# Plachtaa/VALL-E-X

Hardware: AMD Instinct MI355X
Metric: audio-seconds/sec (AR+NAR+Vocos end to end; AR codec-tokens/sec in ar_tokens_per_s), batch32 8s utt (higher is better)
Workload: dtype f32 (cached AR decode step) + f16x2 (operands split into fp16 head + tail = 22 significant bits, tail x tail dropped, fp32 accumulate) for the prefill / NAR projections and full-sequence attention

## Files before the change

### vall-e-x_amd/csrc/engine.hip

```cpp
#include "engine_ctx.h"

#include <deque>
#include <memory>

namespace {
thread_local std::string g_create_err;
}

namespace vxe {

const float* W(vx_ctx* c, const std::string& name) {
  auto it = c->w.find(name);
  return it == c->w.end() ? nullptr : it->second.d;
}

static int ring_slot(vx_ctx* c, size_t n, char** slot) {
  PinRing& r = c->ring;
  if (!r.base) FAIL(VX_ESTATE, "the context has no pinned transfer ring");
  const size_t a = (n + 255) & ~(size_t)255;
  if (r.head + a > r.cap) if (int e = xfer_sync(c)) return e;
  *slot = r.base + r.head;
  r.head += a;
  return VX_OK;
}

int xfer_h2d(vx_ctx* c, void* dst_dev, const void* src_host, size_t bytes) {
  const char* s = static_cast<const char*>(src_host);
  char* d = static_cast<char*>(dst_dev);
  while (bytes) {
    const size_t n = std::min(bytes, XFER_CHUNK);
    char* slot = nullptr;
    if (int e = ring_slot(c, n, &slot)) return e;
    memcpy(slot, s, n);
    HIPCHK(hipMemcpyAsync(d, slot, n, hipMemcpyHostToDevice, c->stream));
    s += n; d += n; bytes -= n;
  }
  return VX_OK;
}

int xfer_d2h(vx_ctx* c, void* dst_host, const void* src_dev, size_t bytes) {
  char* d = static_cast<char*>(dst_host);
  const char* s = static_cast<const char*>(src_dev);
  while (bytes) {
    const size_t n = std::min(bytes, XFER_CHUNK);
    char* slot = nullptr;
    if (int e = ring_slot(c, n, &slot)) return e;
    HIPCHK(hipMemcpyAsync(slot, s, n, hipMemcpyDeviceToHost, c->stream));
    c->ring.pend.push_back({d, slot, n});
    s += n; d += n; bytes -= n;
  }
  return VX_OK;
}

int xfer_sync(vx_ctx* c) {
  const hipError_t e = hipStreamSynchronize(c->stream);
  PinRing& r = c->ring;
  if (e == hipSuccess) {
    size_t total = 0;
    for (const PinRing::Pend& p : r.pend) total += p.n;
    if (total < ((size_t)4 << 20)) {
      for (const PinRing::Pend& p : r.pend) memcpy(p.dst, p.src, p.n);
    } else {
      struct Piece { char* dst; const char* src; size_t n; };
      std::vector<Piece> pieces;
      for (const PinRing::Pend& p : r.pend)
        for (size_t o = 0; o < p.n; o += (size_t)1 << 20)
          pieces.push_back({static_cast<char*>(p.dst) + o, p.src + o, std::min((size_t)1 << 20, p.n - o)});
      constexpr int NT = 4;
      std::thread th[NT - 1];
      auto work = [&pieces](int k) { for (size_t i = k; i < pieces.size(); i += NT) memcpy(pieces[i].dst, pieces[i].src, pieces[i].n); };
      bool started[NT - 1] = {};
      for (int k = 1; k < NT; ++k) {
        try { th[k - 1] = std::thread(work, k); started[k - 1] = true; }
        catch (...) {}
      }
      work(0);
      for (int k = 1; k < NT; ++k) {
        if (started[k - 1]) th[k - 1].join();
        else work(k);
      }
    }
  }
  r.pend.clear();
  r.head = 0;
  HIPCHK(e);
  return VX_OK;
}

int upload_meta(vx_ctx* c) {
  if ((long)c->hmeta.size() > c->imeta_cap) FAIL(VX_EINVAL, "row metadata overflow (%zu > %ld)", c->hmeta.size(), c->imeta_cap);
  H2D(c->imeta, c->hmeta.data(), c->hmeta.size() * sizeof(int));
  return VX_OK;
}

int tap_store(vx_ctx* c, const std::string& name, const float* src, size_t n) {
  if (!c->cfg.debug_taps) return VX_OK;
  Tensor& t = c->taps[name];
  if (t.n < n) {
    void* q = nullptr;
    HIPCHK(hipMalloc(&q, n * sizeof(float)));
    c->allocs.push_back(q);
    t.d = reinterpret_cast<float*>(q);
  }
  t.n = n;
  HIPCHK(hipMemcpyAsync(t.d, src, n * sizeof(float), hipMemcpyDeviceToDevice, c->stream));
  return VX_OK;
}

void gemm(vx_ctx* c, const float* A, int lda, const float* Wt, int ldw, const float* bias, const float* resid, int ldr,
          const float* colscale, float* C, int ldc, long M, int N, int K, int act, const int* gather, int cls, const int* resid_rows) {
  GemmArgs g{};
  g.A = A; g.lda = lda; g.W = Wt; g.ldw = ldw; g.bias = bias; g.resid = resid; g.ldr = ldr; g.colscale = colscale;
  g.C = C; g.ldc = ldc; g.M = (int)M; g.N = N; g.K = K; g.act = act; g.row_gather = gather; g.resid_rows = resid_rows;
  ProfScope ps(c, cls);
  if (c->prof_on) c->prof[cls].bytes += 2.0 * (double)M * N * K;
  launch_gemm_f32(g, c->stream);
}

void proj(vx_ctx* c, const float* A, int lda, const float* Wf, const unsigned short* W3, const float* bias,
          const float* resid, int ldr, float* C, int ldc, long M, int N, int K, int act, const int* gather,
          const unsigned short* a_pre, unsigned short* out_pl, const int* resid_rows) {
  if (c->gemm_mode == 2 || !W3) {
    gemm(c, A, lda, Wf, K, bias, resid, ldr, nullptr, C, ldc, M, N, K, act, gather, 2, resid_rows);
    return;
  }
  const long a_plane = c->gemm_mode == 0 ? h2_plane(M, K, H2_TILE_A) : (long)M * K;
  if (!a_pre) {
    if (c->gemm_mode == 0) launch_split2h(A, lda, M, K, gather, c->fa3, a_plane, H2_TILE_A, c->range_flag, H2_ACT_SCALE, c->stream);
    else launch_split3(A, lda, M, K, gather, c->fa3, a_plane, c->stream);
  }
  GemmX3Args g{};
  g.A = a_pre ? a_pre : c->fa3; g.a_plane = a_plane; g.W = W3; g.w_plane = c->gemm_mode == 0 ? h2_plane(N, K, H2_TILE_W) : (long)N * K;
  g.bias = bias; g.resid = resid; g.ldr = ldr;
  g.colscale = nullptr; g.C = C; g.ldc = ldc; g.M = (int)M; g.N = N; g.K = K; g.act = act;
  g.out_planes = out_pl; g.out_plane = out_pl ? h2_plane(M, N, H2_TILE_A) : 0; g.range_flag = c->range_flag;
  g.resid_rows = resid_rows;
  if (c->gemm_mode == 0) g.descale = ldexpf(1.0f, -(H2_ACT_SHIFT + c->w_shift.at(W3)));
  ProfScope ps(c, 2);
  if (c->prof_on) c->prof[2].bytes += 2.0 * (double)M * N * K;
  if (c->gemm_mode == 0) launch_gemm_f16x2(g, c->stream);
  else if (M >= 1024) launch_gemm_bf16x3_dma(g, c->stream);
  else launch_gemm_bf16x3(g, c->stream);
}


int full_layer(vx_ctx* c, const LayerW& L, long M, const int* seq_off, const int* seq_len, const int* prefix_len,
               int batch, int max_len, const float* ada1, const float* ada2, float* kcl, float* vcl,
               const int* row_b, const int* row_t, double attn_flops, const Trim* tr) {
  const bool pl = c->gemm_mode == 0;
  const long pl1024 = h2_plane(M, D_MODEL, H2_TILE_A);
  launch_layernorm(c->fx, D_MODEL, pl ? nullptr : c->fxn, D_MODEL, (int)M, D_MODEL, LN_EPS, L.n1_w, L.n1_b, ada1,
                   ada1 ? ada1 + D_MODEL : nullptr, c->stream, pl ? c->fa3 : nullptr, pl1024, c->range_flag);
  proj(c, c->fxn, D_MODEL, L.in_w, L.in_w3, L.in_b, nullptr, 0, c->fqkv, 3 * D_MODEL, M, 3 * D_MODEL, D_MODEL, ACT_NONE, nullptr,
       pl ? c->fa3 : nullptr);
  if (kcl) launch_kv_scatter(c->fqkv, row_b, row_t, (int)M, kcl, vcl, c->Tmax, c->stream);
  const bool att_pl = pl && c->attn_x3;
  if (tr && !pl) {
    float* xc = c->fqkv;
    {
      ProfScope ps(c, 3);
      if (c->prof_on) c->prof[3].bytes += tr->attn_flops;
      launch_attn_full(c->fqkv, c->fatt, seq_off, seq_len, prefix_len, batch, max_len, c->stream, tr->q_first, tr->c_off);
    }
    proj(c, c->fatt, D_MODEL, L.out_w, L.out_w3, L.out_b, c->fx, D_MODEL, xc, D_MODEL, tr->Mc, D_MODEL, D_MODEL, ACT_NONE, nullptr, nullptr,
         nullptr, tr->rows);
    launch_layernorm(xc, D_MODEL, c->fxn, D_MODEL, (int)tr->Mc, D_MODEL, LN_EPS, L.n2_w, L.n2_b, ada2, ada2 ? ada2 + D_MODEL : nullptr,
// ... 402 lines not shown
    c->graph_sig = sig;
  }
  hipGraphExec_t& ge = nsteps == 1 ? c->graph_exec : c->graph_exec_n;
  if (!ge) {
    hipGraph_t g = nullptr;
    HIPCHK(hipStreamBeginCapture(c->stream, hipStreamCaptureModeThreadLocal));
    for (int i = 0; i < nsteps; ++i) ar_step_launches(c, sa, rsa);
    HIPCHK(hipStreamEndCapture(c->stream, &g));
    if (int e = launch_status(c)) { (void)hipGraphDestroy(g); return e; }
    HIPCHK(hipGraphInstantiate(&ge, g, nullptr, nullptr, 0));
    (void)hipGraphDestroy(g);
  }
  HIPCHK(hipGraphLaunch(ge, c->stream));
  return VX_OK;
}

bool fb_direct(vx_ctx* c, bool sticky, int& age) {
  if (!sticky || !range_guarded(c)) return false;
  if (++age >= FB_STICKY_PROBE_EVERY) { age = 0; return false; }
  return true;
}
void fb_outcome(vx_ctx* c, bool raised, int& raises, bool& sticky, int& age) {
  if (!range_guarded(c)) return;
  if (!raised) { raises = 0; sticky = false; age = 0; return; }
  if (++raises >= FB_STICKY_AFTER && !sticky) { sticky = true; age = 0; ++c->sticky_engaged; }
}

int ar_generate(vx_ctx* c, const vx_batch* b, const vx_sampling* s, int r0, int nb, std::vector<int>& n_gen,
                std::vector<int>& gen, int beams, unsigned long long seed) {
  const int nb_rows = nb;
  const bool direct_f32 = fb_direct(c, c->sticky_prefill_f32, c->sticky_prefill_age);
  if (direct_f32) {
    ++c->st_fb_prefill; ++c->fb_total;
    if (int e = ensure_f32_buffers(c)) return e;
    F32Scope f32(c);
    if (int e = ar_prefill(c, b, r0, nb_rows, beams)) return e;
  } else if (int e = ar_prefill(c, b, r0, nb_rows, beams)) return e;
  const long ub = (long)b->batch * beams;
  nb = nb_rows * beams;
  if (s->uniforms) {
    const long steps = std::min<long>(s->uniforms_steps, c->gen_stride + 1);
    if (steps * nb > c->uniforms_cap) FAIL(VX_EINVAL, "too many uniforms (%ld steps)", steps);
    std::vector<float> u((size_t)steps * nb);
    for (long t = 0; t < steps; ++t)
      for (int i = 0; i < nb; ++i) u[t * nb + i] = s->uniforms[t * ub + (long)r0 * beams + i];
    H2D(c->d_uniforms, u.data(), u.size() * sizeof(float));
    SYNC();
  }
  H2D(c->seed_dev, &seed, sizeof seed);
  SampleArgs sa = make_sample_args(c, s, 1, nullptr);
  std::vector<int> act(nb);
  bool any = true, raised = false;
  auto first_sample = [&]() -> int {
    int flag = 0;
    HIPCHK(hipMemsetAsync(c->sum_logp, 0, MB * sizeof(float), c->stream));
    LAUNCH(launch_dec_sample(sa, c->stream));
    if (int e = launch_status(c)) return e;
    D2H(act.data(), c->active, nb * sizeof(int));
    if (range_guarded(c) && !direct_f32) D2H(&flag, c->range_flag, sizeof(int));
    SYNC();
    raised = flag != 0;
    any = std::any_of(act.begin(), act.end(), [](int v) { return v != 0; });
    return VX_OK;
  };
  if (int e = first_sample()) return e;
  if (!direct_f32) fb_outcome(c, raised, c->fb_prefill_raises, c->sticky_prefill_f32, c->sticky_prefill_age);
  if (raised) {
    HIPCHK(hipMemsetAsync(c->range_flag, 0, sizeof(int), c->stream));
    ++c->st_fb_prefill; ++c->fb_total;
    if (int e = ensure_f32_buffers(c)) return e;
    {
      F32Scope f32(c);
      if (int e = ar_prefill(c, b, r0, nb_rows, beams)) return e;
      if (int e = first_sample()) return e;
    }
  }
  char sig[160];
  snprintf(sig, sizeof sig, "b%d ns%d c%d%d%d k%d t%a u%d f%d l%d", nb, c->nsplit, (int)c->sb_chain, (int)c->sb_qkv, (int)c->split_fused, sa.top_k, sa.temperature,
           sa.uniforms != nullptr, sa.force_eos_at, sa.sum_logp != nullptr);
  const int sync_every = s->sync_every > 0 ? s->sync_every : 8;
  const int hard_cap = s->force_eos_at >= 0 ? std::min(c->gen_stride + 2, s->force_eos_at) : c->gen_stride + 2;
  int steps = 0;
  const int gs = (c->graph_multi && sync_every % GRAPH_STEPS == 0) ? GRAPH_STEPS : 1;
  while (any && steps < hard_cap) {
    const int n = (steps % gs == 0 && steps + gs <= hard_cap) ? gs : 1;
    if (int e = ar_step_run(c, &sa, sig, n)) return e;
    steps += n;
    if (steps % sync_every == 0) {
      D2H(act.data(), c->active, nb * sizeof(int));
      SYNC();
      any = std::any_of(act.begin(), act.end(), [](int v) { return v != 0; });
    }
  }
  n_gen.resize(nb);
  gen.resize((size_t)nb * c->gen_stride);
  D2H(n_gen.data(), c->n_gen, nb * sizeof(int));
  D2H(gen.data(), c->gen, gen.size() * sizeof(int));
  SYNC();
  c->st_steps += steps;
  if (c->prof_on) {
    for (int i = 0; i < nb; ++i)
      for (int t = 1; t <= n_gen[i]; ++t)
        c->prof[0].bytes += (double)c->NL * ((double)(c->h_L[i] + t) * 2.0 * D_MODEL * 4.0);
    c->prof[1].bytes += (double)steps * ((double)c->NL * 12.0 * D_MODEL * D_MODEL + (double)AR_LOGITS * D_MODEL) * 4.0;
  }
  return VX_OK;
}

static int select_beam(const float* slp, const int* n_gen, int N, int Tp, float length_penalty, bool return_worst) {
  int best = 0, worst = 0;
  double bv = 0, wv = 0;
  for (int j = 0; j < N; ++j) {
    const double len = 1.0 + Tp + n_gen[j];
    const double v = (double)(float)((float)slp[j] / powf((float)len, length_penalty));
    if (j == 0 || v > bv) { bv = v; best = j; }
    if (j == 0 || v < wv) { wv = v; worst = j; }
  }
  return return_worst ? worst : best;
}

static unsigned long long beam_seed(unsigned long long seed, int k) {
  if (k == 0) return seed;
  unsigned long long z = seed + 0x9E3779B97F4A7C15ull * (unsigned long long)k;
  z = (z ^ (z >> 30)) * 0xBF58476D1CE4E5B9ull;
  z = (z ^ (z >> 27)) * 0x94D049BB133111EBull;
  return z ^ (z >> 31);
}

int nar_generate_once(vx_ctx* c, const vx_batch* b, int r0, int nb, const std::vector<int>& T, const int* codes0,
                      long codes0_stride, std::vector<int>& out_codes , long& sumT_out) {
  const int NL = c->NL;
  std::vector<int> seq_off(nb), seq_len(nb), dst_t, id_t, lang_t, pos_t, ycodes, ynj, ydst, ypos, gen_rows, gen_y, q_first(nb), c_off(nb);
  long M = 0, Y = 0, sumT = 0;
  int max_len = 0;
  double trim_attn_flops = 0;
  {
    size_t nS = 0, nY = 0, nT = 0;
    for (int i = 0; i < nb; ++i) { nS += b->text_lens[r0 + i]; nY += b->prompt_lens[r0 + i] + T[i]; nT += T[i]; }
    for (auto* v : {&dst_t, &id_t, &lang_t, &pos_t}) v->reserve(nS);
    for (auto* v : {&ynj, &ydst, &ypos}) v->reserve(nY);
    ycodes.reserve(nY * N_Q);
    gen_rows.reserve(nT); gen_y.reserve(nT);
  }
  for (int i = 0; i < nb; ++i) {
    const int r = r0 + i, S = b->text_lens[r], Tp = b->prompt_lens[r];
    seq_off[i] = (int)M; seq_len[i] = S + Tp + T[i];
    q_first[i] = S + Tp; c_off[i] = (int)sumT;
    trim_attn_flops += 4.0 * T[i] * (double)seq_len[i] * D_MODEL;
    max_len = std::max(max_len, seq_len[i]);
    for (int s = 0; s < S; ++s) {
      dst_t.push_back((int)M + s);
      id_t.push_back(b->text_ids[(long)r * b->text_stride + s]);
      lang_t.push_back(b->text_lang[(long)r * b->text_stride + s]);
      pos_t.push_back(s);
    }
    for (int t = 0; t < Tp + T[i]; ++t) {
      if (t < Tp) {
        for (int j = 0; j < N_Q; ++j) ycodes.push_back(b->prompt_codes[((long)r * b->prompt_stride + t) * N_Q + j]);
        ynj.push_back(N_Q);
      } else {
        ycodes.push_back(codes0[(long)i * codes0_stride + (t - Tp)]);
        for (int j = 1; j < N_Q; ++j) ycodes.push_back(0);
        ynj.push_back(1);
        gen_rows.push_back((int)M + S + t);
        gen_y.push_back((int)Y + t);
      }
      ydst.push_back((int)M + S + t);
      ypos.push_back(t);
    }
    M += seq_len[i]; Y += Tp + T[i]; sumT += T[i];
  }
  sumT_out = sumT;
  out_codes.assign((size_t)(N_Q - 1) * sumT, 0);
  if (sumT == 0) return VX_OK;
// ... 705 lines not shown
}

static int serve_cancel(vx_serve* v, int64_t id, int* state) {
  vx_ctx* c = v->c;
  *state = 0;
  auto wi = std::find_if(v->waiting.begin(), v->waiting.end(), [&](const std::unique_ptr<ServeReq>& q) { return q->id == id; });
  if (wi != v->waiting.end()) {
    v->waiting.erase(wi);
    *state = 1;
    return VX_OK;
  }
  auto li = std::find_if(v->live.begin(), v->live.end(), [&](const std::unique_ptr<ServeReq>& q) { return q->id == id; });
  if (li == v->live.end()) return VX_OK;
  unsigned rows = 0;
  for (int d = 0; d < v->nd; ++d)
    if (v->occ[d] == li->get()) { rows |= 1u << d; v->occ[d] = nullptr; }
  if (rows) launch_serve_cancel(rows, v->nd, c->active, c->slot_meta, c->slot_of, c->n_active, c->stream);
  HIPCHK(hipGetLastError());
  SYNC();
  v->live.erase(li);
  *state = 2;
  return VX_OK;
}

}

extern "C" {

const char* vx_last_error(const vx_ctx* c) { return c ? c->err.c_str() : g_create_err.c_str(); }

int32_t vx_abi_version(void) { return VX_ABI_VERSION; }

int vx_create(int device_id, const vx_config* cfg, vx_ctx** out) {
  if (!cfg || !out) { g_create_err = "null argument"; return VX_EINVAL; }
  if (cfg->struct_size != sizeof(vx_config)) {
    g_create_err = "vx_config.struct_size is " + std::to_string(cfg->struct_size) + ", this library expects " +
                   std::to_string(sizeof(vx_config)) + " (ABI version " + std::to_string(VX_ABI_VERSION) + ")";
    return VX_EINVAL;
  }
  if (cfg->num_layers <= 0 || cfg->max_batch <= 0 || cfg->max_text <= 0 || cfg->max_prompt < 0 || cfg->max_new <= 0) {
    g_create_err = "invalid vx_config";
    return VX_EINVAL;
  }
  int ndev = 0;
  hipError_t e = hipGetDeviceCount(&ndev);
  if (e != hipSuccess || ndev <= 0) {
    g_create_err = std::string("no HIP device available: ") + hipGetErrorString(e);
    return VX_EHIP;
  }
  if (device_id < 0 || device_id >= ndev) { g_create_err = "device_id out of range"; return VX_EINVAL; }
  vx_ctx* c = new vx_ctx();
  c->cfg = *cfg;
  c->dev = device_id;
  c->NL = cfg->num_layers;
  auto fail = [&](hipError_t err, const char* what) {
    g_create_err = std::string(what) + ": " + hipGetErrorString(err);
    delete c;
    return VX_EHIP;
  };
  if ((e = hipSetDevice(device_id)) != hipSuccess) return fail(e, "hipSetDevice");
  bool masked = false;
  for (uint32_t w : cfg->cu_mask) masked |= w != 0;
  if (masked) {
    if ((e = hipExtStreamCreateWithCUMask(&c->stream, 8, cfg->cu_mask)) != hipSuccess)
      return fail(e, "hipExtStreamCreateWithCUMask");
  } else if ((e = hipStreamCreateWithFlags(&c->stream, hipStreamNonBlocking)) != hipSuccess) return fail(e, "hipStreamCreate");
  for (auto& ev : c->ev_t)
    if ((e = hipEventCreate(&ev)) != hipSuccess) {
      for (auto& e2 : c->ev_t) if (e2) (void)hipEventDestroy(e2);
      (void)hipStreamDestroy(c->stream);
      return fail(e, "hipEventCreate");
    }
  {
    size_t mb = 64;
    if (const char* ev = getenv("VX_PIN_MB")) mb = (size_t)std::max(16, std::min(1024, atoi(ev)));
    void* q = nullptr;
    if ((e = hipHostMalloc(&q, mb << 20, hipHostMallocDefault)) != hipSuccess) {
      for (auto& e2 : c->ev_t) if (e2) (void)hipEventDestroy(e2);
      (void)hipStreamDestroy(c->stream);
      return fail(e, "hipHostMalloc (pinned transfer ring)");
    }
    c->ring.base = static_cast<char*>(q);
    c->ring.cap = mb << 20;
  }
  *out = c;
  return VX_OK;
}

void vx_destroy(vx_ctx* c) {
  if (!c) return;
  delete c->serve;
  c->serve = nullptr;
  (void)hipSetDevice(c->dev);
  if (c->stream) (void)hipStreamSynchronize(c->stream);
  if (c->graph_exec) (void)hipGraphExecDestroy(c->graph_exec);
  if (c->graph_exec_n) (void)hipGraphExecDestroy(c->graph_exec_n);
  for (auto& p : c->prof) for (auto ev : p.ev) (void)hipEventDestroy(ev);
  for (auto ev : c->ev_t) if (ev) (void)hipEventDestroy(ev);
  for (void* p : c->allocs) (void)hipFree(p);
  for (auto& kv : c->w) (void)hipFree(kv.second.d);
  if (c->stream) (void)hipStreamDestroy(c->stream);
  if (c->ring.base) (void)hipHostFree(c->ring.base);
  delete c;
}

int vx_synchronize(vx_ctx* c) {
  if (!c) return VX_EINVAL;
  HIPCHK(hipSetDevice(c->dev));
  SYNC();
  return VX_OK;
}

int vx_ar_prefill(vx_ctx* c, const vx_batch* b) {
  if (!c) return VX_EINVAL;
  if (int e = serve_busy(c, "vx_ar_prefill")) return e;
  HIPCHK(hipSetDevice(c->dev));
  if (int e = check_batch(c, b, c->mbr)) return e;
  c->st_fb_prefill = c->st_fb_nar = 0;
  bool raised = fb_direct(c, c->sticky_prefill_f32, c->sticky_prefill_age);
  if (!raised) {
    if (int e = ar_prefill(c, b, 0, b->batch)) return e;
    if (int e = take_range_flag(c, &raised)) return e;
    fb_outcome(c, raised, c->fb_prefill_raises, c->sticky_prefill_f32, c->sticky_prefill_age);
  }
  if (raised) {
    ++c->st_fb_prefill; ++c->fb_total;
    if (int e = ensure_f32_buffers(c)) return e;
    F32Scope f32(c);
    if (int e = ar_prefill(c, b, 0, b->batch)) return e;
  }
  SYNC();
  HIPCHK(hipGetLastError());
  return VX_OK;
}

int vx_ar_logits(vx_ctx* c, float* out) {
  if (!c || !out) return VX_EINVAL;
  if (c->cur_batch <= 0) FAIL(VX_ESTATE, "no prefill has run");
  HIPCHK(hipSetDevice(c->dev));
  SampleArgs sa = make_sample_args(c, nullptr, 0, c->d_logits);
  LAUNCH(launch_dec_sample(sa, c->stream));
  if (int e = launch_status(c)) return e;
  D2H(out, c->d_logits, (size_t)c->cur_batch * AR_LOGITS * sizeof(float));
  SYNC();
  return VX_OK;
}

int vx_ar_step(vx_ctx* c, const int32_t* tokens) {
  if (!c || !tokens) return VX_EINVAL;
  if (int e = serve_busy(c, "vx_ar_step")) return e;
  if (c->cur_batch <= 0) FAIL(VX_ESTATE, "no prefill has run");
  HIPCHK(hipSetDevice(c->dev));
  H2D(c->force_tok, tokens, c->cur_batch * sizeof(int));
  launch_dec_force_token(c->force_tok, c->cur_tok, c->cur_pos, c->ctx_len, c->n_gen, c->gen, c->gen_stride, c->active,
                         c->cur_batch, c->slot_meta, c->slot_of, c->stream);
  if (int e = ar_step_run(c, nullptr, "")) return e;
  SYNC();
  HIPCHK(hipGetLastError());
  return VX_OK;
}

int vx_nar(vx_ctx* c, const vx_batch* b, const int32_t* codes0, int32_t codes0_stride, const int32_t* lens,
           int64_t* out_codes, int32_t out_stride) {
  if (!c || !codes0 || !lens || !out_codes) return VX_EINVAL;
  if (int e = serve_busy(c, "vx_nar")) return e;
  HIPCHK(hipSetDevice(c->dev));
  if (int e = check_batch(c, b, c->mbr)) return e;
  std::vector<int> T(lens, lens + b->batch);
  for (int i = 0; i < b->batch; ++i) {
    if (T[i] < 0 || T[i] > c->cfg.max_new || T[i] > out_stride || T[i] > codes0_stride) FAIL(VX_EINVAL, "row %d: bad length %d", i, T[i]);
    for (int t = 0; t < T[i]; ++t) {
      const int v = codes0[(long)i * codes0_stride + t];
      if (v < 0 || v > AUDIO_VOCAB) FAIL(VX_EINVAL, "row %d: first-codebook id %d out of range (0..1024)", i, v);
    }
  }
  std::vector<int> oc;
  long sumT = 0;
  c->st_fb_prefill = c->st_fb_nar = 0;
  if (int e = nar_generate(c, b, 0, b->batch, T, codes0, codes0_stride, oc, sumT)) return e;
  long off = 0;
  for (int i = 0; i < b->batch; ++i) {
    for (int t = 0; t < T[i]; ++t) {
      int64_t* o = out_codes + ((long)i * out_stride + t) * N_Q;
      o[0] = codes0[(long)i * codes0_stride + t];
      for (int st = 0; st < N_Q - 1; ++st) o[st + 1] = oc[(size_t)st * sumT + off + t];
// ... 271 lines not shown
```

### vall-e-x_amd/csrc/engine_ctx.h

```cpp
#pragma once

#include <math.h>
#include <stdio.h>
#include <stdlib.h>
#include <string.h>

#include <algorithm>
#include <array>
#include <map>
#include <string>
#include <thread>
#include <vector>

#include "../../include/vallex_hip.h"
#include "vx_common.h"

using namespace vx;

namespace vxe {

struct Tensor {
  float* d = nullptr;
  std::vector<int64_t> shape;
  size_t n = 0;
};

struct LayerW {
  const float *in_w, *in_b, *out_w, *out_b, *l1_w, *l1_b, *l2_w, *l2_b, *n1_w, *n1_b, *n2_w, *n2_b;
  float *in_wp = nullptr, *out_wp = nullptr, *l1_wp = nullptr, *l2_wp = nullptr;
  float* out_wh = nullptr;
  unsigned short *in_w3 = nullptr, *out_w3 = nullptr, *l1_w3 = nullptr, *l2_w3 = nullptr;
};

struct PinRing {
  char* base = nullptr;
  size_t cap = 0, head = 0;
  struct Pend { void* dst; const char* src; size_t n; };
  std::vector<Pend> pend;
};
constexpr size_t XFER_CHUNK = 8u << 20;

struct ProfClass {
  std::vector<hipEvent_t> ev;
  size_t used = 0;
  double bytes = 0;
};

constexpr int SK_QKV = 4, SK_OUT = 4, SK_L2 = 8, SK_PRED = 4;
constexpr int PRED_NPAD = 1056;
constexpr int FB_STICKY_AFTER = 2;
constexpr int FB_STICKY_PROBE_EVERY = 32;

}
using namespace vxe;

struct vx_ctx {
  vx_config cfg{};
  int dev = 0;
  hipStream_t stream = nullptr;
  PinRing ring;
  hipEvent_t ev_t[3] = {nullptr, nullptr, nullptr};
  std::string err;
  const char* launch_fail = nullptr;
  std::map<std::string, Tensor> w;
  bool finalized = false;
  std::vector<void*> allocs;

  int NL = 0;
  float* pe = nullptr;
  int pe_rows = 0;
  std::vector<LayerW> ar, nar;
  float* ada = nullptr;
  float* pred_wp = nullptr;
  const float** nar_tabs_dev = nullptr;
  bool has_vocos = false;
  float *vc_embed_w = nullptr, *vc_head_w = nullptr, *vc_head_b = nullptr, *vc_dft = nullptr, *vc_win2 = nullptr;

  int mbr = 0;
  int Tmax = 0;
  long Mmax = 0;

  int gemm_mode = 0;
  bool attn_x3 = true;
  bool attn_h2 = true;
  int* range_flag = nullptr;
  unsigned long long* seed_dev = nullptr;
  int st_fb_prefill = 0, st_fb_nar = 0;
  long fb_total = 0;
  int fb_prefill_raises = 0, fb_nar_raises = 0;
  bool sticky_prefill_f32 = false, sticky_nar_f32 = false;
  int sticky_prefill_age = 0, sticky_nar_age = 0;
  long sticky_engaged = 0;
  unsigned short* fa3b = nullptr;
  unsigned short* fa3 = nullptr;
  unsigned short* pred_w3[N_Q - 1] = {};
  float *fx = nullptr, *fxn = nullptr, *fqkv = nullptr, *fatt = nullptr, *fffn = nullptr, *fyemb = nullptr,
        *flogits = nullptr;
  int* imeta = nullptr;
  long imeta_cap = 0;
  std::vector<int> hmeta;

  float *kc = nullptr, *vc = nullptr;
  float *dh = nullptr, *dh2 = nullptr, *xp = nullptr, *xp_att = nullptr, *xp4 = nullptr;
  bool sb_qkv = false;
  int sb_qkv_rows = 4, sb_qkv_nsplit = 0;
  bool sb_chain = false;
  bool sb_fuse = true;
  bool qkv_bal = true;
  float* qk_new = nullptr;
  float *p_qkv = nullptr, *p_o = nullptr, *p_oh = nullptr, *p_logits = nullptr, *part_o = nullptr, *part_ml = nullptr;
  std::map<const unsigned short*, int> w_shift;
  bool nar_trim = true;
  bool balance_rows = true;
  bool fuse_out = true;
  int fuse_split = 1;
  bool split_fused = false;
  float *d_logits = nullptr, *d_uniforms = nullptr, *sum_logp = nullptr;
  long uniforms_cap = 0;
  int *cur_tok = nullptr, *cur_pos = nullptr, *ctx_len = nullptr, *n_gen = nullptr, *active = nullptr,
      *text_len = nullptr, *gen = nullptr, *force_tok = nullptr, *n_active = nullptr, *slot_meta = nullptr, *slot_of = nullptr;
  int gen_stride = 0;
  int cur_batch = 0;
  int nsplit = 1;
  int att_nsplit_force = 0;
  std::vector<int> h_L;
  vx_serve* serve = nullptr;
  int* row_smp = nullptr;
  int* row_flt = nullptr;

  float* sc_predw = nullptr;
  float* sc_logits = nullptr;
  float* sc_logp = nullptr;
  int* sc_rank = nullptr;

  hipGraphExec_t graph_exec = nullptr, graph_exec_n = nullptr;
  bool graph_multi = true;
  std::string graph_sig;

  std::map<std::string, Tensor> taps;

  int prof_on = 0;
  ProfClass prof[6];
  int64_t st_steps = 0, st_frames = 0;
  int st_truncated = 0;
  double st_ar_ms = 0, st_nar_ms = 0;

  bool has_encodec = false;
  float *ec_codebook = nullptr, *ec_w0 = nullptr, *ec_lstm_b[2] = {nullptr, nullptr}, *ec_whh_p[2] = {nullptr, nullptr};
  float *ec_wT[4] = {}, *ec_bT[4] = {}, *ec_w1[4] = {}, *ec_w3[4] = {};
  float *ec_e0 = nullptr, *ec_x0 = nullptr, *ec_y1 = nullptr, *ec_y2 = nullptr, *ec_xg = nullptr, *ec_col = nullptr,
        *ec_a = nullptr, *ec_sc = nullptr, *ec_out = nullptr, *ec_h = nullptr, *ec_audio = nullptr, *ec_hp = nullptr,
        *ec_c = nullptr, *ec_pg = nullptr;
  long ec_frames_cap = 0;
  bool has_encodec_enc = false;
  float *en_w1[4] = {}, *en_w3[4] = {}, *en_wd[4] = {}, *en_w15 = nullptr, *en_lstm_b[2] = {nullptr, nullptr},
        *en_whh_p[2] = {nullptr, nullptr}, *en_e2 = nullptr, *en_scores = nullptr;
  long long* en_codes = nullptr;

  float *vfeat = nullptr, *vcol = nullptr, *vx0 = nullptr, *vx1 = nullptr, *vhid = nullptr, *vo = nullptr,
        *vreim = nullptr, *vframes = nullptr, *vaudio = nullptr;
  long v_rows_cap = 0;
};

#define HIPCHK(expr)                                                                                   \
  do {                                                                                                 \
    hipError_t _e = (expr);                                                                            \
    if (_e != hipSuccess) {                                                                            \
      char _buf[512];                                                                                  \
      snprintf(_buf, sizeof _buf, "%s failed: %s (%s:%d)", #expr, hipGetErrorString(_e), __FILE__, __LINE__); \
      c->err = _buf;                                                                                   \
      return VX_EHIP;                                                                                  \
    }                                                                                                  \
  } while (0)

#define FAIL(code, ...)                         \
  do {                                          \
    char _buf[512];                             \
    snprintf(_buf, sizeof _buf, __VA_ARGS__);   \
    c->err = _buf;                              \
    return (code);                              \
  } while (0)

#define LAUNCH(call)                                      \
  do {                                                    \
    if (!(call) && !c->launch_fail) c->launch_fail = #call; \
  } while (0)

namespace vxe {

int xfer_h2d(vx_ctx* c, void* dst_dev, const void* src_host, size_t bytes);
int xfer_d2h(vx_ctx* c, void* dst_host, const void* src_dev, size_t bytes);
int xfer_sync(vx_ctx* c);
#define H2D(dst, src, bytes) do { if (int _e = xfer_h2d(c, (dst), (src), (bytes))) return _e; } while (0)
#define D2H(dst, src, bytes) do { if (int _e = xfer_d2h(c, (dst), (src), (bytes))) return _e; } while (0)
#define SYNC() do { if (int _e = xfer_sync(c)) return _e; } while (0)

template <typename T>
int dev_alloc(vx_ctx* c, T** p, size_t count, bool zero = true) {
  void* q = nullptr;
  HIPCHK(hipMalloc(&q, std::max<size_t>(count, 1) * sizeof(T)));
  c->allocs.push_back(q);
  if (zero) HIPCHK(hipMemsetAsync(q, 0, std::max<size_t>(count, 1) * sizeof(T), c->stream));
  *p = reinterpret_cast<T*>(q);
  return VX_OK;
}

const float* W(vx_ctx* c, const std::string& name);

inline int h2_weight_shift(float absmax) {
  if (!(absmax > 0.f) || !(absmax < __builtin_inff())) return 24;
  int ex;
  (void)frexpf(absmax, &ex);
  const int shift = 15 - ex;
  return shift < 0 ? 0 : shift > 24 ? 24 : shift;
}

struct ProfScope {
  vx_ctx* c;
  int which;
  bool on;
  ProfScope(vx_ctx* c_, int w) : c(c_), which(w), on(c_->prof_on == 1 || (c_->prof_on == 2 && w >= 2)) {
    if (!on) return;
    ProfClass& p = c->prof[which];
    if (p.used + 2 > p.ev.size()) {
      for (int i = 0; i < 2; ++i) {
        hipEvent_t e;
        if (hipEventCreate(&e) != hipSuccess) { on = false; return; }
        p.ev.push_back(e);
      }
    }
    (void)hipEventRecord(p.ev[p.used], c->stream);
  }
  ~ProfScope() {
    if (!on) return;
    ProfClass& p = c->prof[which];
    (void)hipEventRecord(p.ev[p.used + 1], c->stream);
    p.used += 2;
  }
};

int upload_meta(vx_ctx* c);

struct MetaBuilder {
  vx_ctx* c;
  explicit MetaBuilder(vx_ctx* c_) : c(c_) { c->hmeta.clear(); }
  long add(const std::vector<int>& v) {
    long off = (long)c->hmeta.size();
    c->hmeta.insert(c->hmeta.end(), v.begin(), v.end());
    while (c->hmeta.size() % 4) c->hmeta.push_back(0);
    return off;
  }
  const int* dev(long off) const { return c->imeta + off; }
};

int tap_store(vx_ctx* c, const std::string& name, const float* src, size_t n);
void gemm(vx_ctx* c, const float* A, int lda, const float* Wt, int ldw, const float* bias, const float* resid, int ldr,
          const float* colscale, float* C, int ldc, long M, int N, int K, int act, const int* gather = nullptr, int cls = 4,
          const int* resid_rows = nullptr);
bool range_guarded(const vx_ctx* c);
int ensure_f32_buffers(vx_ctx* c);
int take_range_flag(vx_ctx* c, bool* raised);
int check_batch(vx_ctx* c, const vx_batch* b, int max_rows);
SampleArgs make_sample_args(vx_ctx* c, const vx_sampling* s, int commit, float* logits_out);
struct ServeSampleArgs;
void ar_step_launches(vx_ctx* c, const SampleArgs* sa, const ServeSampleArgs* rsa = nullptr);
int launch_status(vx_ctx* c);
void decode_geometry(vx_ctx* c, int nrows, bool identity);
void launch_beam_fanout(float* kc, float* vc, long cache_layer, int layers, int Tmax, const int* pairs, int npairs,
                        const float* hsrc, const int* hsrc_row, float* dh, int nrows, hipStream_t s);

struct PrefillPlan {
  int nb = 0, max_len = 0, n_t = 0, n_a = 0;
  long M = 0;
  std::vector<int> seq_off, seq_len, S_;
  std::vector<int> row_b;
  long o_off = 0, o_len = 0, o_S = 0, o_dt = 0, o_it = 0, o_lt = 0, o_pt = 0, o_da = 0, o_ia = 0, o_pa = 0, o_rt = 0, o_rb = 0,
       o_tq = 0, o_tc = 0, o_tr = 0;
// ... 62 lines not shown
```

### vall-e-x_amd/csrc/vocoders.hip

```cpp
#include "engine_ctx.h"

extern "C" {

int vx_vocos_decode(vx_ctx* c, const int64_t* codes, int32_t codes_stride, const int32_t* lens, int32_t batch,
                    int32_t bandwidth_id, float* audio, int64_t audio_stride) {
  if (!c || !codes || !lens || !audio) return VX_EINVAL;
  if (!c->finalized || !c->has_vocos) FAIL(VX_ESTATE, "Vocos weights not loaded");
  if (batch <= 0) FAIL(VX_EINVAL, "bad batch");
  if (bandwidth_id < 0 || bandwidth_id > 3) FAIL(VX_EINVAL, "bandwidth_id must be 0..3");
  HIPCHK(hipSetDevice(c->dev));
  const int C = 384, H = 1152, NBP = 1408, KP = 1312, NF = 1280;
  constexpr int HALO = 32;
  const long cap = c->v_rows_cap;
  struct Job { int row, a, b, lo, hi; };
  std::vector<Job> jobs;
  for (int i = 0; i < batch; ++i) {
    const int T = lens[i];
    if (T < 0 || T > codes_stride) FAIL(VX_EINVAL, "row %d: bad length", i);
    if ((long)T * 320 > audio_stride) FAIL(VX_EINVAL, "audio_stride too small");
    for (long t = 0; t < (long)T * N_Q; ++t) {
      const int64_t v = codes[(long)i * codes_stride * N_Q + t];
      if (v < 0 || v >= AUDIO_VOCAB) FAIL(VX_EINVAL, "code out of range");
    }
    if (T == 0) continue;
    if (T <= cap) { jobs.push_back({i, 0, T, 0, T}); continue; }
    const int Wc = (int)cap - 2 * HALO;
    for (int a = 0; a < T; a += Wc) {
      const int bb = std::min(T, a + Wc);
      jobs.push_back({i, a, bb, std::max(0, a - HALO), std::min(T, bb + HALO)});
    }
  }
  hipStream_t st = c->stream;
  const std::string P = "vocos.backbone.";
  size_t j0 = 0;
  while (j0 < jobs.size()) {
    size_t j1 = j0;
    long R = 0;
    while (j1 < jobs.size() && R + (jobs[j1].hi - jobs[j1].lo) <= cap) { R += jobs[j1].hi - jobs[j1].lo; ++j1; }
    const int nj = (int)(j1 - j0);
    std::vector<int> seq_off(nj), seq_len(nj), row_t, row_len, cd;
    row_t.reserve(R); row_len.reserve(R); cd.reserve(R * N_Q);
    long off = 0;
    int maxT = 0;
    for (int j = 0; j < nj; ++j) {
      const Job& jb = jobs[j0 + j];
      const int T = jb.hi - jb.lo;
      seq_off[j] = (int)off; seq_len[j] = T; maxT = std::max(maxT, T);
      for (int t = 0; t < T; ++t) {
        row_t.push_back(t); row_len.push_back(T);
        for (int q = 0; q < N_Q; ++q) cd.push_back((int)codes[((long)jb.row * codes_stride + jb.lo + t) * N_Q + q]);
      }
      off += T;
    }
    MetaBuilder mb(c);
    const long o_off = mb.add(seq_off), o_len = mb.add(seq_len), o_rt = mb.add(row_t), o_rl = mb.add(row_len), o_cd = mb.add(cd);
    if (int e = upload_meta(c)) return e;
    launch_codebook_sum(mb.dev(o_cd), W(c, "vocos.feature_extractor.codebook_weights"), c->vfeat, (int)R, st);
    launch_im2col7(c->vfeat, 128, mb.dev(o_rt), mb.dev(o_rl), c->vcol, (int)R, st);
    gemm(c, c->vcol, 896, c->vc_embed_w, 896, W(c, P + "embed.bias"), nullptr, 0, nullptr, c->vx0, C, R, C, 896, ACT_NONE);
    launch_layernorm(c->vx0, C, c->vx0, C, (int)R, C, 1e-6f, nullptr, nullptr, W(c, P + "norm.scale.weight") + bandwidth_id * C,
                     W(c, P + "norm.shift.weight") + bandwidth_id * C, st);
    for (int i = 0; i < 8; ++i) {
      const std::string p = P + "convnext." + std::to_string(i) + ".";
      launch_dwconv7(c->vx0, W(c, p + "dwconv.weight"), W(c, p + "dwconv.bias"), mb.dev(o_rt), mb.dev(o_rl), c->vx1, (int)R, C, st);
      launch_layernorm(c->vx1, C, c->vx1, C, (int)R, C, 1e-6f, nullptr, nullptr, W(c, p + "norm.scale.weight") + bandwidth_id * C,
                       W(c, p + "norm.shift.weight") + bandwidth_id * C, st);
      gemm(c, c->vx1, C, W(c, p + "pwconv1.weight"), C, W(c, p + "pwconv1.bias"), nullptr, 0, nullptr, c->vhid, H, R, H, C, ACT_GELU);
      gemm(c, c->vhid, H, W(c, p + "pwconv2.weight"), H, W(c, p + "pwconv2.bias"), c->vx0, C, W(c, p + "gamma"), c->vx0, C, R, C, H,
           ACT_NONE);
    }
    launch_layernorm(c->vx0, C, c->vx1, C, (int)R, C, 1e-6f, W(c, P + "final_layer_norm.weight"), W(c, P + "final_layer_norm.bias"),
                     nullptr, nullptr, st);
    gemm(c, c->vx1, C, c->vc_head_w, C, c->vc_head_b, nullptr, 0, nullptr, c->vo, NBP, R, NBP, C, ACT_NONE);
    launch_istft_prep(c->vo, NBP, c->vreim, KP, (int)R, st);
    gemm(c, c->vreim, KP, c->vc_dft, KP, nullptr, nullptr, 0, nullptr, c->vframes, NF, R, NF, KP, ACT_NONE);
    launch_overlap_add(c->vframes, NF, mb.dev(o_off), mb.dev(o_len), c->vc_win2, c->vaudio, 0, nj, maxT, st);
    for (int j = 0; j < nj; ++j) {
      const Job& jb = jobs[j0 + j];
      D2H(audio + (long)jb.row * audio_stride + (long)jb.a * 320, c->vaudio + ((long)seq_off[j] + (jb.a - jb.lo)) * 320, (size_t)(jb.b - jb.a) * 320 * sizeof(float));
    }
    SYNC();
    HIPCHK(hipGetLastError());
    j0 = j1;
  }
  return VX_OK;
}

int vx_encodec_decode(vx_ctx* c, const int64_t* codes, int32_t codes_stride, const int32_t* lens, int32_t batch,
                      float* audio, int64_t audio_stride) {
  if (!c || !codes || !lens || !audio) return VX_EINVAL;
  if (!c->finalized || !c->has_encodec) FAIL(VX_ESTATE, "EnCodec decoder weights not loaded");
  if (batch <= 0) FAIL(VX_EINVAL, "bad batch");
  HIPCHK(hipSetDevice(c->dev));
  hipStream_t st = c->stream;
  const int ratios[4] = {8, 5, 4, 2};
  for (int r0 = 0; r0 < batch; r0 += c->mbr) {
    const int nb = std::min(c->mbr, batch - r0);
    std::vector<int> seq_off(nb), seq_len(nb), cd;
    long F = 0;
    int maxT = 0;
    for (int i = 0; i < nb; ++i) {
      const int T = lens[r0 + i];
      if (T < 0 || T > c->cfg.max_new || T > codes_stride) FAIL(VX_EINVAL, "row %d: bad length", r0 + i);
      if ((long)T * 320 > audio_stride) FAIL(VX_EINVAL, "audio_stride too small");
      seq_off[i] = (int)F; seq_len[i] = T; maxT = std::max(maxT, T);
      for (int t = 0; t < T; ++t)
        for (int q = 0; q < N_Q; ++q) {
          const int64_t v = codes[((long)(r0 + i) * codes_stride + t) * N_Q + q];
          if (v < 0 || v >= AUDIO_VOCAB) FAIL(VX_EINVAL, "code out of range");
          cd.push_back((int)v);
        }
      F += T;
    }
    if (F == 0) continue;
    if (F > c->ec_frames_cap) FAIL(VX_EINVAL, "too many frames");
    MetaBuilder mb(c);
    const long o_off = mb.add(seq_off), o_len = mb.add(seq_len), o_cd = mb.add(cd);
    if (int e = upload_meta(c)) return e;
    const int* d_off = mb.dev(o_off);
    const int* d_len = mb.dev(o_len);
    launch_codebook_sum(mb.dev(o_cd), c->ec_codebook, c->ec_e0, (int)F, st);
    launch_im2col_seq(c->ec_e0, 128, 7, 0, 0, d_off, d_len, 1, c->ec_col, 896, nb, maxT, st);
    gemm(c, c->ec_col, 896, c->ec_w0, 896, W(c, "encodec.decoder.0.bias"), nullptr, 0, nullptr, c->ec_x0, 512, F, 512, 896,
         ACT_NONE);
    const float* lin = c->ec_x0;
    for (int l = 0; l < 2; ++l) {
      const std::string sfx = "_l" + std::to_string(l);
      gemm(c, lin, 512, W(c, "encodec.decoder.1.lstm.weight_ih" + sfx), 512, c->ec_lstm_b[l], nullptr, 0, nullptr, c->ec_xg,
           2048, F, 2048, 512, ACT_NONE);
      HIPCHK(hipMemsetAsync(c->ec_hp, 0, (size_t)MB * 512 * sizeof(float), st));
      HIPCHK(hipMemsetAsync(c->ec_c, 0, (size_t)MB * 512 * sizeof(float), st));
      float* yout = l == 0 ? c->ec_y1 : c->ec_y2;
      {
        ProfScope ps(c, 5);
        if (c->prof_on) c->prof[5].bytes += (double)maxT;
        for (int t = 0; t < maxT; ++t) {
          launch_skinny_gemm(c->ec_whh_p[l], c->ec_hp, c->ec_pg, 2048, 512, 2, st);
          launch_lstm_cell(c->ec_pg, 2, c->ec_xg, d_off, d_len, t, c->ec_c, c->ec_hp, yout, l == 1 ? c->ec_x0 : nullptr, nb, st);
        }
      }
      lin = yout;
    }
    const float* cur = c->ec_y2;
    int C = 512;
    long R = 1;
    for (int s4 = 0; s4 < 4; ++s4) {
      const int r = ratios[s4], O = C / 2;
      launch_im2col_seq(cur, C, 2, 1, 1, d_off, d_len, (int)R, c->ec_col, 2 * C, nb, (long)maxT * R, st);
      gemm(c, c->ec_col, 2 * C, c->ec_wT[s4], 2 * C, c->ec_bT[s4], nullptr, 0, nullptr, c->ec_a, r * O, F * R, r * O, 2 * C,
           ACT_NONE);
      R *= r;
      C = O;
      const std::string pR = "encodec.decoder." + std::to_string(4 + 3 * s4);
      const long M = F * R;
      const int ldh = std::max(C / 2, 32);
      gemm(c, c->ec_a, C, W(c, pR + ".shortcut.weight"), C, W(c, pR + ".shortcut.bias"), nullptr, 0, nullptr, c->ec_sc, C, M, C,
           C, ACT_NONE);
      launch_im2col_seq(c->ec_a, C, 3, 0, 1, d_off, d_len, (int)R, c->ec_col, 3 * C, nb, (long)maxT * R, st);
      if (ldh != C / 2) HIPCHK(hipMemsetAsync(c->ec_h, 0, (size_t)M * ldh * sizeof(float), st));
      gemm(c, c->ec_col, 3 * C, c->ec_w1[s4], 3 * C, W(c, pR + ".block1.bias"), nullptr, 0, nullptr, c->ec_h, ldh, M, C / 2,
           3 * C, ACT_ELU);
      gemm(c, c->ec_h, ldh, c->ec_w3[s4], ldh, W(c, pR + ".block3.bias"), c->ec_sc, C, nullptr, c->ec_out, C, M, C, ldh,
// ... 109 lines not shown
```

Before: 375.6.

## Overlap EOS polling with AR steps and stream vocoder D2H through event-gated pieces

The AR decode loop no longer stalls the stream on each EOS check. It copies the active flags into one of two pinned slots, records an event, and reads that result only after the next step batch has been enqueued. This keeps the GPU busy at the cost of at most one extra speculative step batch. Vocos audio readback is now split into 1 MB pieces, each with its own event, so host memcpy out of the pinned ring can start while later copies are still in flight. This adds per-piece event creation and synchronisation overhead.

```diff
diff --git a/vall-e-x_amd/csrc/engine.hip b/vall-e-x_amd/csrc/engine.hip
--- a/vall-e-x_amd/csrc/engine.hip
+++ b/vall-e-x_amd/csrc/engine.hip
@@ -22,6 +22,15 @@
   *slot = r.base + r.head;
   r.head += a;
   return VX_OK;
+}
+
+static int ring_fail(vx_ctx* c, hipError_t e, const char* what) {
+  c->ring.pend.clear();
+  c->ring.evs_used = 0;
+  char buf[256];
+  snprintf(buf, sizeof buf, "%s failed: %s (pinned transfer ring)", what, hipGetErrorString(e));
+  c->err = buf;
+  return VX_EHIP;
 }
 
 int xfer_h2d(vx_ctx* c, void* dst_dev, const void* src_host, size_t bytes) {
@@ -32,56 +41,93 @@
     char* slot = nullptr;
     if (int e = ring_slot(c, n, &slot)) return e;
     memcpy(slot, s, n);
-    HIPCHK(hipMemcpyAsync(d, slot, n, hipMemcpyHostToDevice, c->stream));
+    const hipError_t he = hipMemcpyAsync(d, slot, n, hipMemcpyHostToDevice, c->stream);
+    if (he != hipSuccess) return ring_fail(c, he, "hipMemcpyAsync (host to device)");
     s += n; d += n; bytes -= n;
   }
   return VX_OK;
 }
 
-int xfer_d2h(vx_ctx* c, void* dst_host, const void* src_dev, size_t bytes) {
+static int d2h_impl(vx_ctx* c, void* dst_host, const void* src_dev, size_t bytes, size_t piece, bool events) {
   char* d = static_cast<char*>(dst_host);
   const char* s = static_cast<const char*>(src_dev);
+  PinRing& r = c->ring;
   while (bytes) {
-    const size_t n = std::min(bytes, XFER_CHUNK);
+    const size_t n = std::min(bytes, piece);
     char* slot = nullptr;
     if (int e = ring_slot(c, n, &slot)) return e;
-    HIPCHK(hipMemcpyAsync(slot, s, n, hipMemcpyDeviceToHost, c->stream));
-    c->ring.pend.push_back({d, slot, n});
+    hipError_t he = hipMemcpyAsync(slot, s, n, hipMemcpyDeviceToHost, c->stream);
+    if (he != hipSuccess) return ring_fail(c, he, "hipMemcpyAsync (device to host)");
+    int ev = -1;
+    if (events) {
+      if (r.evs_used == r.evs.size()) {
+        hipEvent_t x = nullptr;
+        if ((he = hipEventCreateWithFlags(&x, hipEventDisableTiming)) != hipSuccess) return ring_fail(c, he, "hipEventCreate");
+        r.evs.push_back(x);
+      }
+      ev = (int)r.evs_used++;
+      if ((he = hipEventRecord(r.evs[ev], c->stream)) != hipSuccess) return ring_fail(c, he, "hipEventRecord");
+    }
+    r.pend.push_back({d, slot, n, ev});
     s += n; d += n; bytes -= n;
   }
   return VX_OK;
 }
 
+int xfer_d2h(vx_ctx* c, void* dst_host, const void* src_dev, size_t bytes) {
+  return d2h_impl(c, dst_host, src_dev, bytes, XFER_CHUNK, false);
+}
+
+int xfer_d2h_pieces(vx_ctx* c, void* dst_host, const void* src_dev, size_t bytes) {
+  if (!c->ring.pieces) return xfer_d2h(c, dst_host, src_dev, bytes);
+  return d2h_impl(c, dst_host, src_dev, bytes, XFER_PIECE, true);
+}
+
+static hipError_t ring_deliver(vx_ctx* c, bool with_events) {
+  PinRing& r = c->ring;
+  struct Piece { char* dst; const char* src; size_t n; int ev; };
+  std::vector<Piece> pieces;
+  size_t total = 0;
+  for (const PinRing::Pend& p : r.pend) {
+    if ((p.ev >= 0) != with_events) continue;
+    total += p.n;
+    for (size_t o = 0; o < p.n; o += XFER_PIECE)
+      pieces.push_back({static_cast<char*>(p.dst) + o, p.src + o, std::min(XFER_PIECE, p.n - o), p.ev});
+  }
+  if (pieces.empty()) return hipSuccess;
+  const int NT = total < ((size_t)4 << 20) ? 1 : 4;
+  hipError_t err[4] = {hipSuccess, hipSuccess, hipSuccess, hipSuccess};
+  auto work = [&](int k) {
+    if (with_events && k) (void)hipSetDevice(c->dev);
+    for (size_t i = k; i < pieces.size(); i += NT) {
+      const Piece& q = pieces[i];
+      if (q.ev >= 0 && err[k] == hipSuccess) err[k] = hipEventSynchronize(r.evs[q.ev]);
+      if (err[k] == hipSuccess) memcpy(q.dst, q.src, q.n);
+    }
+  };
+  std::thread th[3];
+  bool started[3] = {};
+  for (int k = 1; k < NT; ++k) {
+    try { th[k - 1] = std::thread(work, k); started[k - 1] = true; }
+    catch (...) {}
+  }
+  work(0);
+  for (int k = 1; k < NT; ++k) {
+    if (started[k - 1]) th[k - 1].join();
+    else work(k);
+  }
+  for (hipError_t e : err) if (e != hipSuccess) return e;
+  return hipSuccess;
+}
+
 int xfer_sync(vx_ctx* c) {
-  const hipError_t e = hipStreamSynchronize(c->stream);
   PinRing& r = c->ring;
-  if (e == hipSuccess) {
-    size_t total = 0;
-    for (const PinRing::Pend& p : r.pend) total += p.n;
-    if (total < ((size_t)4 << 20)) {
-      for (const PinRing::Pend& p : r.pend) memcpy(p.dst, p.src, p.n);
-    } else {
-      struct Piece { char* dst; const char* src; size_t n; };
-      std::vector<Piece> pieces;
-      for (const PinRing::Pend& p : r.pend)
-        for (size_t o = 0; o < p.n; o += (size_t)1 << 20)
-          pieces.push_back({static_cast<char*>(p.dst) + o, p.src + o, std::min((size_t)1 << 20, p.n - o)});
-      constexpr int NT = 4;
-      std::thread th[NT - 1];
-      auto work = [&pieces](int k) { for (size_t i = k; i < pieces.size(); i += NT) memcpy(pieces[i].dst, pieces[i].src, pieces[i].n); };
-      bool started[NT - 1] = {};
-      for (int k = 1; k < NT; ++k) {
-        try { th[k - 1] = std::thread(work, k); started[k - 1] = true; }
-        catch (...) {}
-      }
-      work(0);
-      for (int k = 1; k < NT; ++k) {
-        if (started[k - 1]) th[k - 1].join();
-        else work(k);
-      }
-    }
-  }
+  hipError_t e = ring_deliver(c, true);
+  const hipError_t es = hipStreamSynchronize(c->stream);
+  if (e == hipSuccess) e = es;
+  if (e == hipSuccess) e = ring_deliver(c, false);
   r.pend.clear();
+  r.evs_used = 0;
   r.head = 0;
   HIPCHK(e);
   return VX_OK;
@@ -650,14 +696,26 @@
   const int hard_cap = s->force_eos_at >= 0 ? std::min(c->gen_stride + 2, s->force_eos_at) : c->gen_stride + 2;
   int steps = 0;
   const int gs = (c->graph_multi && sync_every % GRAPH_STEPS == 0) ? GRAPH_STEPS : 1;
-  while (any && steps < hard_cap) {
-    const int n = (steps % gs == 0 && steps + gs <= hard_cap) ? gs : 1;
-    if (int e = ar_step_run(c, &sa, sig, n)) return e;
-    steps += n;
-    if (steps % sync_every == 0) {
-      D2H(act.data(), c->active, nb * sizeof(int));
-      SYNC();
-      any = std::any_of(act.begin(), act.end(), [](int v) { return v != 0; });
+  int slot = 0, pending = -1;
+  while (true) {
+    const bool run = any && steps < hard_cap;
+    if (run) {
+      const int n = (steps % gs == 0 && steps + gs <= hard_cap) ? gs : 1;
+      if (int e = ar_step_run(c, &sa, sig, n)) return e;
+      steps += n;
+    }
+    if (pending >= 0 && run) {
+      HIPCHK(hipEventSynchronize(c->poll_ev[pending]));
+      const int* f = c->poll_pin + pending * MB;
+      any = std::any_of(f, f + nb, [](int v) { return v != 0; });
+      pending = -1;
+    }
+    if (!run || !any) break;
+    if (steps % sync_every == 0 && steps < hard_cap) {
+      HIPCHK(hipMemcpyAsync(c->poll_pin + slot * MB, c->active, nb * sizeof(int), hipMemcpyDeviceToHost, c->stream));
+      HIPCHK(hipEventRecord(c->poll_ev[slot], c->stream));
+      pending = slot;
+      slot ^= 1;
     }
   }
   n_gen.resize(nb);
@@ -1529,6 +1587,25 @@
     }
     c->ring.base = static_cast<char*>(q);
     c->ring.cap = mb << 20;
+    if (const char* ev = getenv("VX_D2H_PIECES")) c->ring.pieces = atoi(ev) != 0;
+  }
+  {
+    void* q = nullptr;
+    e = hipHostMalloc(&q, 2 * MB * sizeof(int), hipHostMallocDefault);
+    if (e == hipSuccess) {
+      c->poll_pin = static_cast<int*>(q);
+      memset(q, 0, 2 * MB * sizeof(int));
+      for (auto& ev : c->poll_ev)
+        if (e == hipSuccess) e = hipEventCreateWithFlags(&ev, hipEventDisableTiming);
+    }
+    if (e != hipSuccess) {
+      for (auto& e2 : c->poll_ev) if (e2) (void)hipEventDestroy(e2);
+      if (c->poll_pin) (void)hipHostFree(c->poll_pin);
+      for (auto& e2 : c->ev_t) if (e2) (void)hipEventDestroy(e2);
+      (void)hipStreamDestroy(c->stream);
+      (void)hipHostFree(c->ring.base);
+      return fail(e, "hipHostMalloc / hipEventCreate (EOS poll slots)");
+    }
   }
   *out = c;
   return VX_OK;
@@ -1547,7 +1624,11 @@
   for (void* p : c->allocs) (void)hipFree(p);
   for (auto& kv : c->w) (void)hipFree(kv.second.d);
   if (c->stream) (void)hipStreamDestroy(c->stream);
+  c->ring.pend.clear();
+  for (auto ev : c->ring.evs) (void)hipEventDestroy(ev);
   if (c->ring.base) (void)hipHostFree(c->ring.base);
+  for (auto ev : c->poll_ev) if (ev) (void)hipEventDestroy(ev);
+  if (c->poll_pin) (void)hipHostFree(c->poll_pin);
   delete c;
 }
 
diff --git a/vall-e-x_amd/csrc/engine_ctx.h b/vall-e-x_amd/csrc/engine_ctx.h
--- a/vall-e-x_amd/csrc/engine_ctx.h
+++ b/vall-e-x_amd/csrc/engine_ctx.h
@@ -35,10 +35,14 @@
 struct PinRing {
   char* base = nullptr;
   size_t cap = 0, head = 0;
-  struct Pend { void* dst; const char* src; size_t n; };
+  struct Pend { void* dst; const char* src; size_t n; int ev; };
   std::vector<Pend> pend;
+  std::vector<hipEvent_t> evs;
+  size_t evs_used = 0;
+  bool pieces = true;
 };
 constexpr size_t XFER_CHUNK = 8u << 20;
+constexpr size_t XFER_PIECE = 1u << 20;
 
 struct ProfClass {
   std::vector<hipEvent_t> ev;
@@ -60,6 +64,8 @@
   hipStream_t stream = nullptr;
   PinRing ring;
   hipEvent_t ev_t[3] = {nullptr, nullptr, nullptr};
+  int* poll_pin = nullptr;
+  hipEvent_t poll_ev[2] = {nullptr, nullptr};
   std::string err;
   const char* launch_fail = nullptr;
   std::map<std::string, Tensor> w;
@@ -190,9 +196,11 @@
 
 int xfer_h2d(vx_ctx* c, void* dst_dev, const void* src_host, size_t bytes);
 int xfer_d2h(vx_ctx* c, void* dst_host, const void* src_dev, size_t bytes);
+int xfer_d2h_pieces(vx_ctx* c, void* dst_host, const void* src_dev, size_t bytes);
 int xfer_sync(vx_ctx* c);
 #define H2D(dst, src, bytes) do { if (int _e = xfer_h2d(c, (dst), (src), (bytes))) return _e; } while (0)
 #define D2H(dst, src, bytes) do { if (int _e = xfer_d2h(c, (dst), (src), (bytes))) return _e; } while (0)
+#define D2H_PIECES(dst, src, bytes) do { if (int _e = xfer_d2h_pieces(c, (dst), (src), (bytes))) return _e; } while (0)
 #define SYNC() do { if (int _e = xfer_sync(c)) return _e; } while (0)
 
 template <typename T>
diff --git a/vall-e-x_amd/csrc/vocoders.hip b/vall-e-x_amd/csrc/vocoders.hip
--- a/vall-e-x_amd/csrc/vocoders.hip
+++ b/vall-e-x_amd/csrc/vocoders.hip
@@ -77,7 +77,7 @@
     launch_overlap_add(c->vframes, NF, mb.dev(o_off), mb.dev(o_len), c->vc_win2, c->vaudio, 0, nj, maxT, st);
     for (int j = 0; j < nj; ++j) {
       const Job& jb = jobs[j0 + j];
-      D2H(audio + (long)jb.row * audio_stride + (long)jb.a * 320, c->vaudio + ((long)seq_off[j] + (jb.a - jb.lo)) * 320, (size_t)(jb.b - jb.a) * 320 * sizeof(float));
+      D2H_PIECES(audio + (long)jb.row * audio_stride + (long)jb.a * 320, c->vaudio + ((long)seq_off[j] + (jb.a - jb.lo)) * 320, (size_t)(jb.b - jb.a) * 320 * sizeof(float));
     }
     SYNC();
     HIPCHK(hipGetLastError());
```

Result: no change. 377.1, median of 4 (+0.4%).
